# WCC-Analytics/sidecar

Measured on AMD Instinct MI355X. Metric: record-merges/sec (whole node) + rounds-to-converge wall time, H=32768 S=16, higher is better.
Workload: dtype int64

## Files before the change

sidecar_amd/csrc/gx_device.hpp:

```cpp
#pragma once
#include <hip/hip_runtime.h>
#include <stdint.h>

#include "../../include/gx.h"

#define GXD __device__ __forceinline__
#define GXHD __host__ __device__ __forceinline__

#define GX_GLOBAL __attribute__((address_space(1)))
typedef unsigned int gx_u32x4 __attribute__((ext_vector_type(4)));
template <class T>
GXD T gld(const T *p) {
  return *(const GX_GLOBAL T *)p;
}
typedef unsigned int gx_u32x3 __attribute__((ext_vector_type(3)));
template <class T>
GXD void gst(T *p, T v) {
  *(GX_GLOBAL T *)p = v;
}
GXD gx_u32x4 gld4(const void *p) { return *(const GX_GLOBAL gx_u32x4 *)p; }
GXD gx_u32x3 gld3(const void *p) { return *(const GX_GLOBAL gx_u32x3 *)p; }
GXD void gst4(void *p, gx_u32x4 v) { *(GX_GLOBAL gx_u32x4 *)p = v; }

struct grec {
// ... 51 lines not shown

struct Dev {
  gx_params p;
  int64_t epoch;
  uint32_t H, S, R, Q, A, L, SQ, DQ, K;
  uint32_t NG, KE;
  uint32_t KG;
  uint32_t lo, Hl, G, gid;
  uint32_t n_remote;
  uint32_t *msg_key;
  uint32_t *in_stamp;
  int64_t round, now;
  int partitioned;
  uint64_t *view;
  unsigned long long *minexp;
  uint8_t *own_status;
  gx_host_state *hs;
  gx_job *fifo;
  gx_sleeper *sleep;
  grec *dq;
  grec *arena;
  uint32_t *arena_len;
  uint32_t AW;
  uint32_t *arena_bits;
  grec *msg;
  uint64_t *msg_w0;
  uint32_t *msg_len;
  uint32_t *msg_dst;
  uint32_t DI;
  uint32_t DR;
  uint32_t *in_cnt;
  uint32_t *in_cnt_nx;
  uint4 *in_hdr;
  uint4 *in_ovf;
  grec *in_rec;
  uint32_t *work_cnt;
  uint32_t *wl_cnt, *wl_cnt_nx;
  uint32_t *ovf_cnt, *ovf_cnt_nx;
  uint32_t *work;
  uint32_t *mrec;
  grec *scan_list;
  uint32_t *scan_cnt;
  uint8_t *tick;
  uint16_t *sbytes;
  gx_server_times *srvt;
  int64_t *vlc;
  int32_t *ev_slot;
  gx_change_event *ev_log;
  uint32_t *ev_cnt;
  uint32_t ev_cap;
  DevCtr *ctr;
  gx_member *mem;
  int32_t *fd_dl;
  gx_fd_host *fdh;
  gx_fd_msg *fdm;
  uint32_t *fd_len;
  uint32_t *fd_peers;
  uint32_t *fd_np;
  uint64_t *fd_snap;
  int pair_split;
  uint64_t divS;
  uint32_t logS;
  int departures;
  uint32_t nblk_ae;
  uint64_t *snap;
  uint32_t snap_tag, snap_word;
// ... 145 lines not shown
    atomicMin(&d.ctr->first_drop[shard_id()][1], (unsigned long long)d.round);
}

GXD uint32_t li(const Dev &d, uint32_t v) { return v - d.lo; }
GXD uint32_t owner_of(const Dev &d, uint32_t r) { return d.S == 1 ? r : (uint32_t)__umul64hi(d.divS, (uint64_t)r); }
GXD bool owned_by(const Dev &d, uint32_t r, uint32_t o) { return r - o * d.S < d.S; }
GXD bool departed(const Dev &d, uint32_t u) { return d.departures && departed_at(d.p, d.round, u); }

GXD void wave_sync() {
  __builtin_amdgcn_fence(__ATOMIC_SEQ_CST, "wavefront");
  __builtin_amdgcn_wave_barrier();
}

#define GX_ERR_INBOX 1u
#define GX_WC_ERR 4
#define GX_WC_SCANS 5
#define GX_WC_N 8
#define GX_SNAP_QUIET 0xffffffffu
GXD uint32_t inbox_claim(const Dev &d, uint32_t vi) { return atomicAdd(&d.in_cnt[vi], 1u); }
GXD void inbox_header(const Dev &d, uint32_t vi, uint32_t pos, uint32_t key, uint32_t entry, uint32_t len,
                      uint32_t slot) {
  if (pos < d.DI) d.in_hdr[(size_t)vi * d.DI + pos] = make_uint4(key, entry, len, slot);
  else d.in_ovf[atomicAdd(d.ovf_cnt, 1u)] = make_uint4(key, entry, len, vi);
}
GXD void inbox_header(const Dev &d, uint32_t vi, uint32_t pos, uint32_t key, uint32_t entry, uint32_t len) {
  inbox_header(d, vi, pos, key, entry, len, pos);
}
GXD void inbox_put(const Dev &d, uint32_t vi, uint32_t key, uint32_t entry, uint32_t len) {
  inbox_header(d, vi, inbox_claim(d, vi), key, entry, len);
}
GXD grec *packet_recs(const Dev &d, uint32_t vi, uint32_t slot, uint32_t entry) {
  return slot < d.DR ? &d.in_rec[((size_t)vi * d.DR + slot) * d.p.packet_cap] : &d.msg[(size_t)entry * d.p.packet_cap];
}
GXD uint4 inbox_next(const Dev &d, uint32_t vi, int64_t after) {
  uint4 best = make_uint4(0xffffffffu, 0u, 0u, 0u);
  bool found = false;
  const uint32_t cnt = d.in_cnt[vi], n = cnt < d.DI ? cnt : d.DI;
  for (uint32_t i = 0; i < n; i++) {
    const uint4 h = d.in_hdr[(size_t)vi * d.DI + i];
    if ((int64_t)h.x > after && (!found || h.x < best.x)) {
      best = h;
      found = true;
    }
  }
  const uint32_t no = *d.ovf_cnt;
  for (uint32_t i = 0; i < no; i++) {
    const uint4 h = d.in_ovf[i];
    if (h.w == vi && (int64_t)h.x > after && (!found || h.x < best.x)) {
      best = make_uint4(h.x, h.y, h.z, 0xffffffffu);
      found = true;
    }
  }
  return best;
}
GXD void flag_live(const Dev &d, uint32_t vi, uint32_t n) { atomicAdd(&d.mrec[vi], n); }
GXD gx_member *memp(const Dev &d, uint32_t v, uint32_t m) { return &d.mem[(size_t)li(d, v) * d.H + m]; }
GXD int32_t *dlp(const Dev &d, uint32_t v, uint32_t m) { return &d.fd_dl[(size_t)li(d, v) * d.H + m]; }
GXD gx_fd_host *fdhp(const Dev &d, uint32_t v) { return &d.fdh[li(d, v)]; }
GXD bool reach(const Dev &d, uint32_t a, uint32_t b) {
  if (departed(d, a) || departed(d, b)) return false;
  return !(d.partitioned && ((a < d.H / 2) != (b < d.H / 2)));
}
GXD uint64_t *vrow(const Dev &d, uint32_t v) { return &d.view[(size_t)li(d, v) * d.R]; }
GXD gx_host_state *hst(const Dev &d, uint32_t v) { return &d.hs[li(d, v)]; }

GXD void set_slot(const Dev &d, Acc &a, uint32_t v, uint64_t *slot, uint64_t nw) {
  if (*slot != nw) {
    *slot = nw;
    a.changed = true;
    atomicMin(&d.minexp[li(d, v)], exp_time(d.p, nw));
  }
}

GXD bool locked_in(const Dev &d, uint32_t lockw) { return GX_LOCK_AT(lockw, d.round) != 0u; }
GXD bool host_locked(const Dev &d, uint32_t v) { return locked_in(d, gld(&hst(d, v)->lock)); }
GXD uint32_t lock_snap(uint32_t lockw, uint32_t flags, int64_t round, bool rw) {
  const uint32_t b = 1u << (round & 1), w = 16u << (round & 1);
  lockw = (lockw & ~b) | ((flags & 3u) ? b : 0u);
  return rw ? (lockw & ~w) | ((flags & 2u) ? w : 0u) : lockw;
}
#define GX_NOHOST 0xffffffffu
#define GX_LOCK_READERS_CLAIMED 2u
GXD bool ro_side(const Dev &d, uint32_t v) {
  const gx_host_state *h = hst(d, v);
  const uint32_t lw = gld(&h->lock);
// ... 608 lines not shown
```

sidecar_amd/csrc/gx_engine.hip:

```cpp
#include <hip/hip_runtime.h>

#include <math.h>
#include <stdio.h>
#include <stdlib.h>
#include <string.h>

#include <algorithm>
#include <chrono>
#include <deque>
#include <numeric>
#include <string>
#include <thread>
#include <type_traits>
#include <vector>


#define HIPCHK(x)                                                                          \
  do {                                                                                     \
    hipError_t _e = (x);                                                                   \
    if (_e != hipSuccess) {                                                                \
      fprintf(stderr, "gx: HIP error %s at %s:%d\n", hipGetErrorString(_e), __FILE__, __LINE__); \
      return GX_EIO;                                                                       \
    }                                                                                      \
  } while (0)
// ... 1030 lines not shown
  d.L = p->packet_cap + p->pending_cap;
  d.K = p->fanout;
  d.NG = p->gossip_messages > 1 ? p->gossip_messages : 1;
  d.KG = d.K * d.NG;
  d.KE = d.KG + (p->probe_piggyback ? 2u : 0u);
  d.divS = d.S > 1 ? ~0ull / d.S + 1 : 0;
  while ((1u << d.logS) < d.S) d.logS++;
  d.G = p->n_shards > 1 ? p->n_shards : 1;
  d.gid = d.G > 1 ? p->shard_id : 0;
  d.lo = (uint32_t)(((uint64_t)d.gid * d.H) / d.G);
  d.Hl = (uint32_t)(((uint64_t)(d.gid + 1) * d.H) / d.G) - d.lo;
  d.SQ = pow2_at_least(64 > d.KE * (p->retransmit_rounds + 1) ? 64 : d.KE * (p->retransmit_rounds + 1));
  d.DQ = pow2_at_least(d.L + p->pending_cap + 64);
  d.nblk_ae = (d.R + GX_DIGEST_SLOTS - 1) / GX_DIGEST_SLOTS;
  d.DI = p->inbox_slots ? p->inbox_slots : (d.NG > 1 ? GX_DI_MAX : 64);
  d.DR = d.DI < 8 ? d.DI : 8;
  d.sfilt = 1u;
  d.QW = 4 * nblk(d.Hl ? d.Hl : 1, 64);
  d.departures = p->depart_round >= 0 && p->depart_ppm;
  if (p->lock_model) {
    d.C = p->lock_buffer;
    d.PW = (d.H + 31) / 32;
    if (p->lock_readers) d.P = p->lock_defer_slots ? p->lock_defer_slots : 64;
    if (p->fd_handoff_shared) d.HQ = d.C > GX_LOCK_HANDLER_AT ? d.C - GX_LOCK_HANDLER_AT : 0;
  }
  e->scan_nch = 1;
  if (d.R >= 65536 && d.S >= 2 && 128 % d.S == 0)
    e->scan_nch = d.R / 32768 < 16 ? d.R / 32768 : 16;
  if (getenv("GX_KPROF"))
    e->kprof_n = (size_t)nblk(d.Hl, 64) * 4 * 8 + GX_KPROF_MERGE_N + 3ull * d.H;
  if (const char *qs = getenv("GX_QUIET_SEND")) e->quiet_send = strcmp(qs, "0") != 0;
  e->quiet_batch = GX_QUIET_BATCH;
  if (const char *qb = getenv("GX_QUIET_BATCH")) e->quiet_batch = (uint32_t)std::min(std::max(atol(qb), 1l), 1024l);
  if (d.G > 1) {
    e->nblk = d.nblk_ae;
    e->nmw = (e->nblk + 31) / 32;
  }
}

static int create_streams(gx_engine *e) {
  HIPCHK(hipStreamCreateWithFlags(&e->own_stream, hipStreamNonBlocking));
  e->stream = e->own_stream;
  HIPCHK(hipStreamCreateWithFlags(&e->side_stream, hipStreamNonBlocking));
  HIPCHK(hipEventCreateWithFlags(&e->side_start, hipEventDisableTiming));
  HIPCHK(hipEventCreateWithFlags(&e->side_done, hipEventDisableTiming));
  HIPCHK(hipHostMalloc((void **)&e->scan_snap, (2 + GX_QUIET_SLOTS) * sizeof(uint64_t), hipHostMallocMapped));
  HIPCHK(hipHostGetDevicePointer((void **)&e->scan_snap_dev, e->scan_snap, 0));
  e->scan_snap[0] = e->scan_snap[1] = ~0ull;
  for (int i = 0; i < GX_QUIET_SLOTS; i++) e->scan_snap[2 + i] = 0;
  return GX_OK;
}

#define DERIVED 0u
#define TAKE(...) GXTRY(e->mem.take(__VA_ARGS__))

static int create_buffers(gx_engine *e) {
  Dev &d = e->d;
  const gx_params *p = &d.p;
  hipStream_t s = e->stream;
  const size_t Hg = d.H, H = d.Hl, K = d.KE ? d.KE : 1;
  TAKE(GX_CK_VIEW, d.view, sizeof(uint64_t) * H * d.R);
  TAKE(GX_CK_OWN_STATUS, d.own_status, H * d.S);
  TAKE(GX_CK_HS, d.hs, sizeof(gx_host_state) * H);
  TAKE(GX_CK_FIFO, d.fifo, sizeof(gx_job) * H * d.Q);
  TAKE(GX_CK_SLEEP, d.sleep, sizeof(gx_sleeper) * H * d.SQ);
  TAKE(GX_CK_DQ, d.dq, sizeof(grec) * H * d.DQ);
  TAKE(GX_CK_ARENA, d.arena, sizeof(grec) * H * d.A * d.L);
  TAKE(GX_CK_ARENA_LEN, d.arena_len, sizeof(uint32_t) * H * d.A, 0, s);
  TAKE(GX_CK_ARENA_BITS, d.arena_bits, sizeof(uint32_t) * H * d.AW);
  TAKE(GX_CK_MSG, d.msg, sizeof(grec) * Hg * K * p->packet_cap);
  TAKE(GX_CK_MSG_W0, d.msg_w0, sizeof(uint64_t) * Hg * K * p->packet_cap);
  TAKE(GX_CK_MSG_LEN, d.msg_len, sizeof(uint32_t) * Hg * K, 0, s);
  TAKE(GX_CK_MSG_DST, d.msg_dst, sizeof(uint32_t) * Hg * K);
  TAKE(GX_CK_MSG_KEY, d.msg_key, sizeof(uint32_t) * Hg * K);
  TAKE(GX_CK_IN_CNT, e->in_cnt_buf, sizeof(uint32_t) * 2 * H, 0, s);
  TAKE(GX_CK_IN_HDR, d.in_hdr, sizeof(uint4) * H * d.DI);
  TAKE(GX_CK_IN_OVF, d.in_ovf, sizeof(uint4) * Hg * K);
  TAKE(GX_CK_IN_REC, d.in_rec, sizeof(grec) * H * d.DR * p->packet_cap);
  TAKE(GX_CK_WORK_CNT, d.work_cnt, sizeof(uint32_t) * GX_WC_N, 0, s);
  TAKE(DERIVED, d.quiet_w, sizeof(uint32_t) * 2 * d.QW, 0, s);
  TAKE(GX_CK_WORK, d.work, sizeof(uint32_t) * H);
  if (p->push_pull_mode == GX_PP_INITIATE && d.G < 2) {
    TAKE(DERIVED, e->pp_dev, sizeof(uint32_t) * 2 * Hg);
    TAKE(DERIVED, e->pp_prow, sizeof(int32_t) * Hg, 0xff, s);
  }
  TAKE(GX_CK_MREC, d.mrec, sizeof(uint32_t) * H, 0, s);
  TAKE(GX_CK_MINEXP, d.minexp, sizeof(unsigned long long) * H);
  TAKE(GX_CK_SCAN_LIST, d.scan_list, sizeof(grec) * H * d.L);
  TAKE(GX_CK_SCAN_CNT, d.scan_cnt, sizeof(uint32_t) * H);
  if (e->scan_nch > 1) {
    TAKE(DERIVED, e->scan_tmp, sizeof(grec) * H * e->scan_nch * d.L);
    TAKE(DERIVED, e->scan_chunk, sizeof(ScanChunk) * H * e->scan_nch);
  }
  TAKE(GX_CK_TICK, d.tick, H, 0, s);
  TAKE(GX_CK_SBYTES, d.sbytes, sizeof(uint16_t) * d.R);
  TAKE(GX_CK_SRVT, d.srvt, sizeof(gx_server_times) * H * Hg);
  TAKE(GX_CK_VLC, d.vlc, sizeof(int64_t) * H);
  TAKE(DERIVED, d.ev_slot, sizeof(int32_t) * H, 0xff, s);
  TAKE(GX_CK_CTR, d.ctr, sizeof(DevCtr), 0, s);
  if (p->fd_enable) {
    TAKE(GX_CK_MEM, d.mem, sizeof(gx_member) * H * Hg);
    TAKE(GX_CK_FD_DL, d.fd_dl, sizeof(int32_t) * H * Hg);
    TAKE(GX_CK_FDH, d.fdh, sizeof(gx_fd_host) * H);
    TAKE(GX_CK_FDM, d.fdm, sizeof(gx_fd_msg) * Hg * K * p->fd_msg_cap);
    TAKE(GX_CK_FD_LEN, d.fd_len, sizeof(uint32_t) * Hg * K, 0, s);
    TAKE(GX_CK_FD_PEERS, d.fd_peers, sizeof(uint32_t) * H * K);
    TAKE(GX_CK_FD_NP, d.fd_np, sizeof(uint32_t) * H);
    if (p->fd_push_pull_state) TAKE(GX_CK_FD_SNAP, d.fd_snap, sizeof(uint64_t) * H * Hg);
  }
// ... 394 lines not shown
```

sidecar_amd/csrc/gx_kernels.hpp:

```cpp
#pragma once
#include "gx_device.hpp"

GXD unsigned long long block_excl_scan64(unsigned long long x, unsigned long long *s_wave,
                                         unsigned long long &total) {
  uint32_t lane = threadIdx.x & 63, w = threadIdx.x >> 6, nw = (blockDim.x + 63) >> 6;
  unsigned long long incl = x;
  for (int o = 1; o < 64; o <<= 1) {
    unsigned long long y = __shfl_up(incl, o, 64);
    if ((int)lane >= o) incl += y;
  }
  if (lane == 63) s_wave[w] = incl;
  __syncthreads();
  unsigned long long off = 0, tot = 0;
  for (uint32_t i = 0; i < nw; i++) {
    unsigned long long c = s_wave[i];
    if (i < w) off += c;
    tot += c;
  }
  __syncthreads();
  total = tot;
  return off + incl - x;
}
GXD uint32_t fld(unsigned long long x, int i) { return (uint32_t)((x >> (16 * i)) & 0xffffu); }

// ... 1296 lines not shown
GXD uint32_t shard_of_d(const Dev &d, uint32_t v) {
  uint32_t g = (uint32_t)(((uint64_t)v * d.G) / d.H);
  while (g > 0 && (uint32_t)(((uint64_t)g * d.H) / d.G) > v) g--;
  while (g + 1 < d.G && (uint32_t)(((uint64_t)(g + 1) * d.H) / d.G) <= v) g++;
  return g;
}
GXD uint32_t *ob_slot_hdr(const Dev &d, uint32_t slot) {
  return reinterpret_cast<uint32_t *>(d.ob_buf + (size_t)slot * (16u + 16u * d.p.packet_cap));
}
static_assert(sizeof(PlanCall) >= 17 * sizeof(uint32_t), "a PlanCall slot holds a team's 16 peers and their count");
#define GX_NOSLOT 0xffffffffu
#define GX_NOSLOT_W0 0xfffffffeu
GXD bool w0_fwd(const Dev &d, uint32_t slot, uint32_t tick, uint32_t key, uint32_t v) {
  return slot == GX_NOSLOT_W0 && tick != 2 && !owned_by(d, key, v);
}

GXD grec plan_item(const Dev &d, const PlanCall &c, uint32_t i) {
  grec g;
  g.pad = 0;
  if (c.kind == GX_JOB_SEND) {
    const grec s = c.list[i];
    g.w = s.w + c.bw;
    g.r = s.r;
  } else if (c.kind == GX_JOB_EXPIRE) {
    g.w = c.bw;
    g.r = c.rb + (c.emask ? nth_set_bit(c.emask, i) : i);
  } else {
    g.w = c.bw;
    g.r = c.rb;
  }
  return g;
}

template <int T, bool QUIET = false>
GXD void send_planned(const Dev &d, Acc &a, uint32_t idx, gx_host_state &hs, gx_job *pjs, PlanCall *pl,
                      const uint32_t *peers, uint32_t np, unsigned long long &kb, unsigned long long &kl,
                      uint32_t npf0 = 0) {
  constexpr int PLAN_Q = PLAN_RECS / T;
  const uint32_t lane = threadIdx.x & 63, tl = lane & (T - 1), tw = lane / T;
  const bool lead = tl == 0;
  const uint64_t tmask = T == 64 ? ~0ull : ((1ull << T) - 1ull);
  const uint32_t u = d.lo + idx, cap = d.p.packet_cap, mask = d.DQ - 1;
  grec *dq = &d.dq[(size_t)idx * d.DQ];
  grec *const arena_t = &d.arena[(size_t)idx * d.A * d.L];
  grec *const msg_t = &d.msg[(size_t)idx * d.KE * cap];
  uint64_t *const w0_t = &d.msg_w0[(size_t)idx * d.KE * cap];
  const int64_t t_stale = d.now - d.p.tombstone_lifespan_ns - d.p.stale_fudge_ns;
  const int64_t t_gc = d.now - d.p.tombstone_lifespan_ns;
  uint32_t pf0 = hs.fifo_head, npf = npf0;
  uint32_t j = 0, n = 0;
  bool stop = np == 0;
  unsigned fm = 0, fs = 0, nlines = 0;
  GX_SPLIT_DECL
  const bool lmod = QUIET || d.p.lock_model != 0;
  constexpr int NR = (16 + T - 1) / T;
  const bool direct = !QUIET && d.ob_buf != nullptr;
  uint32_t osl[NR];
  uint32_t emit = 0;
#pragma unroll
  for (int r = 0; r < NR; r++) osl[r] = GX_NOSLOT;
  uint32_t og[NR], rk[NR], ksrc[NR], krun[NR], lc[NR], lb[NR], le[NR];
  if (direct) {
    unsigned long long pend[NR];
#pragma unroll
    for (int r = 0; r < NR; r++) {
      const uint32_t jj = (uint32_t)r * T + tl;
      og[r] = jj < np && peers[jj] - d.lo >= d.Hl ? shard_of_d(d, peers[jj]) : d.G;
      pend[r] = __ballot(og[r] < d.G);
      rk[r] = ksrc[r] = krun[r] = lc[r] = 0;
    }
    for (;;) {
      int r0 = -1;
#pragma unroll
      for (int r = NR - 1; r >= 0; r--) r0 = pend[r] ? r : r0;
      if (r0 < 0) break;
      unsigned long long p0 = pend[0];
      uint32_t g0 = og[0];
#pragma unroll
      for (int r = 1; r < NR; r++) {
        p0 = r == r0 ? pend[r] : p0;
        g0 = r == r0 ? og[r] : g0;
      }
      const uint32_t src = (uint32_t)__builtin_ctzll(p0);
      const uint32_t gs = (uint32_t)__shfl((int)g0, (int)src, 64);
      uint32_t acc = 0;
#pragma unroll
      for (int r = 0; r < NR; r++) {
// ... 149 lines not shown
        const uint32_t nn = c.m + hs.dq_len;
        l = nn < cap ? nn : cap;
        c.head = hs.dq_head;
        if (l < c.m) {
          c.push = c.m - l;
          c.nh = (c.head - c.push) & mask;
          any_push = true;
        } else {
          c.nh = (c.head + (l - c.m)) & mask;
        }
        hs.dq_head = c.nh;
        hs.dq_len = nn - l;
        if (hs.dq_len > d.p.pending_cap) {
          if (lead) a.c[C_PDROP] += hs.dq_len - d.p.pending_cap;
          hs.dq_len = d.p.pending_cap;
        }
        if (l && lead) {
          a.c[C_PACKETS]++;
          a.c[C_RECSENT] += l;
          const uint32_t lb = l < c.m ? l : c.m;
          const bool filt = c.row && !(lmod && c.lk);
          if (c.lk & 2u) {
            a.c[C_LOCK_DROP] += l;
          } else {
            kb += 16ull * ((c.kind == GX_JOB_SEND ? lb : 0u) + (l - lb)) + (filt ? 8ull * l : 0ull);
          }
          if (filt) fm += l;
          if (c.lk) {
            a.locked = true;
            if (!lmod) a.c[C_LOCKED_MERGES] += l;
          }
        }
      }
      c.l = l;
      c.lpre = tot;
      if (l) {
        if (c.oslot != GX_NOSLOT) emit |= 1u << j;
        if constexpr (QUIET) {
          if (c.push) cp = c;
        } else {
          if (lead) pl[nc] = c;
        }
        nc++;
        if (!(c.lk & 2u)) tot += l;
      }
      const bool pushed = c.push != 0;
      if (l == 0) {
        if (n == 0 && d.p.gossip_stop_on_empty) stop = true;
        j++;
        n = 0;
      } else if (++n == d.NG) {
        j++;
        n = 0;
      }
      if (j >= np) stop = true;
      if (pushed) break;
    }
    if (nc == 0) break;
    if constexpr (QUIET) {
#ifndef GX_SEND_SPLIT
      if (j <= PLAN_CH) {
        GX_KP(5);
        GX_KP(6);
      }
#endif
      GX_SPLIT(0);
      for (uint32_t qq = (tl - cp.nh) & (T - 1); qq < cp.push; qq += T) {
        dq[(cp.nh + qq) & mask] = plan_item(d, cp, cp.l + qq);
        kb += 16;
      }
      GX_SPLIT(3);
      continue;
    }
    wave_sync();
#ifndef GX_SEND_SPLIT
    if (j <= PLAN_CH) GX_KP(5);
#endif
// ... 91 lines not shown
        }
        if (live) {
          grec g;
          g.w = w[q];
          g.r = r[q];
          g.pad = 0;
          const uint32_t xo = (c.x - idx * d.KE) * cap + rank;
          grec *to = c.oslot != GX_NOSLOT ? reinterpret_cast<grec *>(ob_slot_hdr(d, c.oslot) + 4) + rank : &msg_t[xo];
          gst_rec(to, g);
          if (filt) gst(&w0_t[xo], w0[q]);
        }
        run += (uint32_t)__popcll(lm);
      }
    }
#pragma unroll
    for (int kk = 1; kk < PLAN_CH; kk++)
      if (lp[kk] == tot) cb[kk] = run;
    uint32_t stored_all = 0;
#ifndef GX_SEND_SPLIT
    if (j <= PLAN_CH) GX_KP(6);
#endif
    GX_SPLIT(1);
    if (tl < nc) {
      const PlanCall &c = pl[tl];
      uint32_t stored = 0;
#pragma unroll
      for (int kk = 0; kk < PLAN_CH; kk++) {
        const uint32_t end = kk + 1 < PLAN_CH && (uint32_t)(kk + 1) < nc ? cb[kk + 1] : run;
        stored = (uint32_t)kk == tl ? end - cb[kk] : stored;
      }
      const uint32_t rv = c.peer - d.lo;
      if (!c.row) stored = c.l;
      if (c.lk & 2u) stored = 0;
      d.msg_len[c.x] = stored;
      d.msg_dst[c.x] = c.peer;
      if (c.oslot != GX_NOSLOT)
        *reinterpret_cast<uint4 *>(ob_slot_hdr(d, c.oslot)) = make_uint4(c.key, c.peer, stored, 0u);
      if (c.row && stored) {
        inbox_header(d, rv, inbox_claim(d, rv), c.key, c.x, stored, lmod && c.lk ? GX_NOSLOT : GX_NOSLOT_W0);
        flag_live(d, rv, stored);
      }
      stored_all = stored + ((c.row && stored) ? 2u : 0u);
    }
    kb += 16ull * stored_all;
    GX_SPLIT(2);
    if (any_push) {
      for (uint32_t k = 0; k < nc; k++) {
        const PlanCall &c = pl[k];
        for (uint32_t qq = (tl - c.nh) & (T - 1); qq < c.push; qq += T) {
          dq[(c.nh + qq) & mask] = plan_item(d, c, c.l + qq);
          kb += 16;
        }
      }
      __threadfence_block();
    }
    wave_sync();
    GX_SPLIT(3);
  }
  GX_SPLIT_FLUSH();
#pragma unroll
  for (int r = 0; r < NR; r++)
    if (osl[r] != GX_NOSLOT && !((emit >> ((uint32_t)r * T + tl)) & 1u))
      *reinterpret_cast<uint4 *>(ob_slot_hdr(d, osl[r])) = make_uint4(GX_SLOT_EMPTY, 0u, 0u, 0u);
  a.c[C_GOSSIP_MERGES] += fm;
  kl += nlines;
  a.c[C_STALE] += fs;
}

GXD bool filt_used(const Dev &d, uint32_t pos) { return d.sfilt && pos != 0xffffffffu; }
#define PLAN_PEERS(QUIET) ((QUIET) ? 0 : PLAN_CH)
template <int T, bool FWD, int SW>
GXD uint32_t quiet_tick(const Dev &d, Acc &a, uint32_t idx, gx_host_state &hs, gx_sleeper *sj, gx_job *pj,
                        uint32_t *peers) {
  const uint32_t tl = threadIdx.x & (T - 1), o = d.lo + idx;
  const bool lead = tl == 0;
// ... 400 lines not shown
      const unsigned long long n = wave_sum((unsigned long long)cross[c]);
      if ((threadIdx.x & 63) == 0 && n) atomicAdd(&d.probe_x[c], n);
    }
  }
}

template <bool K32>
GXD uint64_t bitonic64(uint64_t x, uint32_t lane) {
#pragma unroll
  for (uint32_t k = 2; k <= 64; k <<= 1) {
#pragma unroll
    for (uint32_t j = k >> 1; j > 0; j >>= 1) {
      uint64_t o;
      if (K32) o = (uint32_t)__shfl_xor((uint32_t)x, (int)j, 64);
      else o = __shfl_xor(x, (int)j, 64);
      bool keep_min = ((lane & j) == 0) == ((lane & k) == 0);
      x = keep_min ? (o < x ? o : x) : (o > x ? o : x);
    }
  }
  return x;
}

GXD uint32_t rdl(uint32_t x, uint32_t l) { return (uint32_t)__builtin_amdgcn_readlane((int)x, (int)l); }

GXD void merge_inbox_serial(const Dev &d, uint32_t vi, bool lockd = false, uint32_t nbuf = 0) {
  Acc a;
  const uint32_t v = d.lo + vi, cnt = d.in_cnt[vi];
  int64_t after = -1;
  unsigned long long recs = 0;
  grec *lkb = d.lkb ? &d.lkb[(size_t)vi * d.C] : nullptr;
  if (lockd) {
    uint32_t nb = GX_LOCK_BUF(d.hs[vi].lock);
    const uint32_t capv = pipe_cap(d, vi, d.hs[vi].lock);
    for (uint32_t n = 0; n < cnt; n++) {
      const uint4 h = inbox_next(d, vi, after);
      after = h.x;
      const grec *pk = packet_recs(d, vi, h.w, h.y);
      for (uint32_t x = 0; x < h.z; x++) {
        if (nb < capv) {
          lkb[nb++] = pk[x];
          a.c[C_LOCK_BUF]++;
        } else {
          a.c[C_LOCK_DROP]++;
        }
      }
      recs += h.z;
    }
    d.hs[vi].lock = (d.hs[vi].lock & ((1u << GX_LOCK_BUF_SHIFT) - 1u)) | nb << GX_LOCK_BUF_SHIFT;
    kbytes(d, GX_K_MERGE, 32ull * recs + 16ull * cnt + 4, 0);
    for (int i = 0; i < C_NCTR; i++) ctr_atomic(d, i, a.c[i]);
    return;
  }
  for (uint32_t k = 0; k < nbuf; k++) add_entry(d, a, v, lkb[k], SRC_GOSSIP);
  const unsigned m0 = a.c[C_GOSSIP_MERGES], s0 = a.c[C_STALE];
  if (nbuf) {
    a.c[C_LOCK_DRAIN] += nbuf;
    d.hs[vi].lock &= (1u << GX_LOCK_BUF_SHIFT) - 1u;
  }
  for (uint32_t n = 0; n < cnt; n++) {
    const uint4 h = inbox_next(d, vi, after);
    after = h.x;
    const grec *pk = packet_recs(d, vi, h.w, h.y);
    for (uint32_t x = 0; x < h.z; x++) add_entry(d, a, v, pk[x], SRC_GOSSIP);
    recs += h.z;
  }
  recs += nbuf;
  a.c[C_GOSSIP_MERGES] = m0;
  a.c[C_STALE] = s0;
  kbytes(d, GX_K_MERGE, 28ull * recs + 16ull * cnt + 4, recs);
  for (int i = 0; i < C_NCTR; i++) ctr_atomic(d, i, a.c[i]);
  if (a.changed) mark_change(d);
}

#define INBOX_PREFETCH 8
#define MERGE_WAVES 4
#define MSET 512
#define MSET_EMPTY 0xffffffffu
GXD uint32_t mset_slot(uint32_t key) { return (key * 0x9E3779B1u) >> (32 - 9); }
GXD bool mset_has(const uint32_t *set, uint32_t key) {
  for (uint32_t h = mset_slot(key), n = 0; n < MSET; n++, h = (h + 1) & (MSET - 1)) {
    const uint32_t x = set[h];
    if (x == key) return true;
// ... 10 lines not shown
struct MergeLds {
  uint4 hdr[GX_DI_MAX];
  uint32_t pst[GX_DI_MAX];
  uint64_t accw[64];
  uint32_t wset[MSET];
  uint8_t accf[64], chg[64], prev[64];
};
template <bool K32, bool EV>
GXD void merge_receiver(const Dev &d, const uint32_t vi, MergeLds &L) {
  uint4 *s_hdr = L.hdr;
  uint8_t *s_accf = L.accf, *s_chg = L.chg, *s_prev = L.prev;
  uint64_t *s_accw = L.accw;
  const uint32_t lane = threadIdx.x & 63, v = d.lo + vi;
  const uint32_t npre = d.DI < INBOX_PREFETCH ? d.DI : INBOX_PREFETCH;
  uint4 hd = lane < npre ? d.in_hdr[(size_t)vi * d.DI + lane] : make_uint4(0u, 0u, 0u, 0u);
  const uint32_t deg = d.in_cnt[vi];
  uint32_t lw = 0, nbuf = 0;
  bool lockd = false;
  if (d.p.lock_model) {
    lw = __builtin_amdgcn_readfirstlane(d.hs[vi].lock);
    lockd = locked_in(d, lw);
    nbuf = lockd || departed(d, v) ? 0u : GX_LOCK_BUF(lw);
  }
  if (deg == 0 && nbuf == 0) return;
  if (deg > d.DI) {
    if (lane == 0) merge_inbox_serial(d, vi, lockd, nbuf);
    return;
  }
  const bool wide = deg > 64;
  uint4 sh = make_uint4(0u, 0u, 0u, 0u);
  uint32_t pstart = 0, total = 0;
  if (!wide) {
    if (deg > npre && lane >= npre && lane < deg) hd = d.in_hdr[(size_t)vi * d.DI + lane];
    const uint32_t hkey = lane < deg ? hd.x : 0xffffffffu;
    uint32_t hrank = 0;
    for (uint32_t j = 0; j < deg; j++) hrank += rdl(hkey, j) < hkey || (rdl(hkey, j) == hkey && j < lane);
    if (lane < deg) s_hdr[hrank] = hd;
    wave_sync();
    sh = lane < deg ? s_hdr[lane] : make_uint4(0u, 0u, 0u, 0u);
    uint32_t incl = sh.z;
#pragma unroll
    for (int o = 1; o < 64; o <<= 1) {
      uint32_t y = __shfl_up(incl, o, 64);
      if ((int)lane >= o) incl += y;
    }
    pstart = incl - sh.z;
    total = __shfl(incl, 63, 64);
  } else {
    constexpr int HPL = GX_DI_MAX / 64;
    uint4 hw[HPL];
#pragma unroll
    for (int c = 0; c < HPL; c++) {
      const uint32_t j = lane + 64u * c;
      hw[c] = j < deg ? (j < npre ? hd : d.in_hdr[(size_t)vi * d.DI + j]) : make_uint4(0u, 0u, 0u, 0u);
      if (j < deg) L.pst[j] = hw[c].x;
    }
    wave_sync();
    uint32_t rk[HPL];
#pragma unroll
    for (int c = 0; c < HPL; c++) rk[c] = 0;
    for (uint32_t j = 0; j < deg; j++) {
      const uint32_t kj = L.pst[j];
#pragma unroll
      for (int c = 0; c < HPL; c++) {
        const uint32_t me = lane + 64u * c;
        rk[c] += kj < hw[c].x || (kj == hw[c].x && j < me);
      }
    }
#pragma unroll
    for (int c = 0; c < HPL; c++)
      if (lane + 64u * c < deg) s_hdr[rk[c]] = hw[c];
    wave_sync();
    for (uint32_t c0 = 0; c0 < deg; c0 += 64) {
      const uint32_t j = c0 + lane;
      const uint32_t ln = j < deg ? s_hdr[j].z : 0u;
      uint32_t incl = ln;
#pragma unroll
      for (int o = 1; o < 64; o <<= 1) {
        uint32_t y = __shfl_up(incl, o, 64);
        if ((int)lane >= o) incl += y;
      }
      if (j < deg) L.pst[j] = total + incl - ln;
      total += __shfl(incl, 63, 64);
    }
    wave_sync();
  }
  const uint32_t vtick = d.tick[vi];
// ... 14 lines not shown
  }
  const grec *lkb = nbuf ? &d.lkb[(size_t)vi * d.C] : nullptr;
  const uint32_t ntot = nbuf + total;
  auto load_recs = [&](uint32_t tb, grec &g, uint32_t &fslot, uint64_t &fw0) {
    uint32_t i = tb + lane;
    g.w = 0;
    g.r = INV;
    g.pad = 0;
    fw0 = 0;
    fslot = 0;
    if (i < nbuf) {
      g = gld_rec(&lkb[i]);
      return;
    }
    i -= nbuf;
    if (i < total) {
      uint32_t lo = 0, hi = deg;
      while (hi - lo > 1) {
        const uint32_t mid = (lo + hi) >> 1;
        if (L.pst[mid] <= i) lo = mid;
        else hi = mid;
      }
      const uint4 hk = s_hdr[lo];
      const uint32_t off = i - L.pst[lo];
      fslot = hk.w;
      g = packet_recs(d, vi, hk.w, hk.y)[off];
      if (hk.w == GX_NOSLOT_W0) fw0 = d.msg_w0[(size_t)hk.y * d.p.packet_cap + off];
    }
  };
  if (lockd) {
    const uint32_t capv = pipe_cap(d, vi, lw), nb0 = GX_LOCK_BUF(lw), room_l = capv > nb0 ? capv - nb0 : 0u;
    const uint32_t keep = total < room_l ? total : room_l;
    grec *dst = &d.lkb[(size_t)vi * d.C + nb0];
    for (uint32_t t0 = 0; t0 < keep; t0 += 64) {
      grec g;
      uint32_t fs;
      uint64_t fw;
      load_recs(t0, g, fs, fw);
      if (t0 + lane < keep) gst_rec(&dst[t0 + lane], g);
    }
    if (lane == 0) {
      d.hs[vi].lock = (lw & ((1u << GX_LOCK_BUF_SHIFT) - 1u)) | (nb0 + keep) << GX_LOCK_BUF_SHIFT;
      ctr_atomic(d, C_LOCK_BUF, keep);
      ctr_atomic(d, C_LOCK_DROP, total - keep);
      kbytes(d, GX_K_MERGE, 32ull * keep + 16ull * deg + 4, 0);
    }
    wave_sync();
    return;
  }
  const bool track = ntot > 64;
  if (track)
    for (uint32_t q = lane; q < MSET; q += 64) L.wset[q] = MSET_EMPTY;
  uint32_t nset = 0;
  grec gc, gn;
  uint32_t fsc, fsn = 0;
  uint64_t fwc, fwn = 0;
  load_recs(0, gc, fsc, fwc);
  gn.w = 0;
  gn.r = INV;
  gn.pad = 0;
  if (64 < ntot) load_recs(64, gn, fsn, fwn);
  wave_sync();
  unsigned long long *kpm = kprof_merge(d);
  unsigned long long ph[5] = {0, 0, 0, 0, 0}, tk = 0;
  uint32_t c_dstale = 0;
  for (uint32_t t0 = 0; t0 < ntot; t0 += 64) {
    if (kpm) tk = __builtin_amdgcn_s_memtime();
    const uint32_t i = t0 + lane;
    const bool valid = i < ntot;
    uint32_t key = INV;
    uint64_t val = 0, w0 = 0;
    bool rd = false;
    if (valid) {
      key = gc.r;
      val = gc.w;
      bool fwd = w0_fwd(d, fsc, vtick, key, v);
      if (fwd && t0 > 0) fwd = nset <= MSET / 2 && !mset_has(L.wset, key);
      rd = !fwd;
// ... 350 lines not shown
    const uint32_t ok = n_retx < room ? n_retx : room;
    if (n_retx) {
      d.hs[vi].fifo_tail = tail0 + n_retx;
      d.hs[vi].fifo_stored = st0 + ok;
    }
    if (mcmax) d.vlc[vi] = ts_of(s_accw[mcmax - 1]);
    if (EV && evk >= 0) d.ev_cnt[evk] = ev0 + n_ev;
    ctr_atomic(d, C_CHG, c_chg);
    kbytes(d, GX_K_MERGE, 12ull * total + 8ull * (total + c_wr) + 16ull * ok + 16ull * deg + 4, total);
    ctr_atomic(d, C_GOSSIP_ACC, c_acc);
    ctr_atomic(d, C_RETX, n_retx);
    ctr_atomic(d, C_QDEFER, n_retx - ok);
    if (c_wr) {
      mark_change(d);
      atomicMin(&d.minexp[vi], mexp);
    }
  }
  wave_sync();
  return true;
}

#ifndef MERGE_WPE_GM
#define MERGE_WPE_GM 4
#endif
#ifndef LOCK_RPL
#define LOCK_RPL 4
#endif
template <int SEG>
GXD bool lock_append_seg(const Dev &d, uint32_t vi, bool act) {
  const uint32_t lane = threadIdx.x & 63, sl = lane & (SEG - 1), sb = lane & ~(uint32_t)(SEG - 1);
  const uint32_t deg = act ? d.in_cnt[vi] : 0u;
  const uint32_t lw = act ? d.hs[vi].lock : 0u;
  uint4 hd = d.in_hdr[(size_t)vi * d.DI + (sl < d.DI ? sl : 0u)];
  if (deg > (uint32_t)SEG || deg > d.DI) return false;
  if (sl >= deg) hd = make_uint4(0xffffffffu, 0u, 0u, 0u);
  uint32_t start = 0, total = 0;
  for (uint32_t j = 0; j < (uint32_t)SEG; j++) {
    const uint32_t kj = (uint32_t)__shfl((int)hd.x, (int)(sb + j), 64);
    const uint32_t lj = (uint32_t)__shfl((int)hd.z, (int)(sb + j), 64);
    const bool before = j < deg && (kj < hd.x || (kj == hd.x && j < sl));
    start += before ? lj : 0u;
    total += j < deg ? lj : 0u;
  }
  const uint32_t capv = pipe_cap(d, vi, lw), nb0 = GX_LOCK_BUF(lw), room = capv > nb0 ? capv - nb0 : 0u;
  const uint32_t keep = total < room ? total : room;
  grec *dst = act ? &d.lkb[(size_t)vi * d.C + nb0] : d.lkb;
  for (uint32_t o0 = 0; o0 < keep; o0 += SEG * LOCK_RPL) {
    grec g[LOCK_RPL];
#pragma unroll
    for (int q = 0; q < LOCK_RPL; q++) {
      const uint32_t o = o0 + sl + SEG * q;
      uint32_t entry = 0, slot = 0, off = 0;
      for (uint32_t j = 0; j < deg; j++) {
        const uint32_t sj = (uint32_t)__shfl((int)start, (int)(sb + j), 64);
        const uint32_t lj = (uint32_t)__shfl((int)hd.z, (int)(sb + j), 64);
        const uint32_t ej = (uint32_t)__shfl((int)hd.y, (int)(sb + j), 64);
        const uint32_t wj = (uint32_t)__shfl((int)hd.w, (int)(sb + j), 64);
        if (o >= sj && o < sj + lj) {
          entry = ej;
          slot = wj;
          off = o - sj;
        }
      }
      g[q] = gld_rec(&packet_recs(d, vi, slot, entry)[off]);
    }
#pragma unroll
    for (int q = 0; q < LOCK_RPL; q++) {
      const uint32_t o = o0 + sl + SEG * q;
      if (o < keep) gst_rec(&dst[o], g[q]);
    }
  }
  if (act && sl == 0 && deg) {
    d.hs[vi].lock = (lw & ((1u << GX_LOCK_BUF_SHIFT) - 1u)) | (nb0 + keep) << GX_LOCK_BUF_SHIFT;
    ctr_atomic(d, C_LOCK_BUF, keep);
    ctr_atomic(d, C_LOCK_DROP, total - keep);
    kbytes(d, GX_K_MERGE, 32ull * keep + 16ull * deg + 4, 0);
  }
  return true;
}

#ifndef GX_LOCK_APPEND_WPE
#define GX_LOCK_APPEND_WPE 8
#endif
__global__ __launch_bounds__(256) __attribute__((amdgpu_waves_per_eu(GX_LOCK_APPEND_WPE))) void k_lock_append(Dev d) {
  const uint32_t vi = (blockIdx.x * 256u + threadIdx.x) >> 4;
  bool act = false;
  if (vi < d.Hl) act = d.mrec[vi] != 0 && locked_in(d, d.hs[vi].lock);
  if (__ballot(act) == 0) return;
  const bool ok = lock_append_seg<16>(d, act ? vi : 0u, act);
  if (act && ok && (threadIdx.x & 15) == 0) d.mrec[vi] = 0;
}

#define MERGE_NR 64
#define MERGE_NONE 0xffffffffu
template <bool K32, bool EV, int NR = MERGE_NR, int WPE = 3>
__global__ __launch_bounds__(64 * MERGE_WAVES) __attribute__((amdgpu_waves_per_eu(WPE))) void k_merge_seg(Dev d) {
  static_assert(NR <= 64, "one routing lane per receiver");
  __shared__ MergeLds s_l[MERGE_WAVES];
  __shared__ uint32_t s_it[NR][4];
  __shared__ uint32_t s_ty[NR];
  __shared__ uint32_t s_fb[NR], s_n[2];
  const uint32_t wv = threadIdx.x >> 6, lane = threadIdx.x & 63;
  const uint32_t r0 = blockIdx.x * NR;
  if (wv == 0) {
    const uint32_t vi = r0 + lane;
    uint32_t t = 0;
    if (lane < (uint32_t)NR && vi < d.Hl) t = d.mrec[vi];
    if (t) d.mrec[vi] = 0;
    if (lane < (uint32_t)NR)
// ... 2156 lines not shown
```

Before: 4.153 billion.

## Send compact packet descriptors for lock-buffered expire/retx records instead of full records

Result: no change. 4.114 billion (-0.9%).

```diff
diff --git a/profiles/lock_desc/pmc_sum.py b/profiles/lock_desc/pmc_sum.py
--- /dev/null
+++ b/profiles/lock_desc/pmc_sum.py
@@ -0,0 +1,28 @@
+import csv
+import json
+import sys
+
+FIRST, LAST = 9, 28
+
+if __name__ == "__main__":
+    label, counter, path = sys.argv[1:4]
+    rows = {}
+    with open(path) as f:
+        for r in csv.DictReader(f):
+            if r["Counter_Name"] == counter:
+                k = int(r["Dispatch_Id"])
+                name, v = rows.get(k, (r["Kernel_Name"], 0.0))
+                rows[k] = (name, v + float(r["Counter_Value"]))
+    scale = 1024.0 * (2 if counter == "FETCH_SIZE" else 1)
+    rnd, out = -1, {"k_send": [0, 0.0], "k_lock_append": [0, 0.0]}
+    for k in sorted(rows):
+        name, v = rows[k]
+        if "k_send" in name:
+            rnd += 1
+        base = "k_send" if "k_send" in name else "k_lock_append" if "k_lock_append" in name else None
+        if base and FIRST <= rnd <= LAST:
+            out[base][0] += 1
+            out[base][1] += v * scale
+    print(json.dumps({"lib": label, "counter": counter, "rounds": f"{FIRST}..{LAST}",
+                      **{k: {"launches": n, "MB": round(b / 1e6, 2), "MB_per_launch": round(b / 1e6 / max(1, n), 3)}
+                         for k, (n, b) in out.items()}}))
diff --git a/profiles/lock_desc/rounds.py b/profiles/lock_desc/rounds.py
--- /dev/null
+++ b/profiles/lock_desc/rounds.py
@@ -0,0 +1,12 @@
+import os
+import sys
+
+sys.path.insert(0, os.getcwd())
+import bench
+from sidecar_amd.abi import load_product
+
+if __name__ == "__main__":
+    e = bench.make_engine(load_product(), "cfg5", 0x5EED, 0)
+    for _ in range(int(sys.argv[1])):
+        e.run_rounds(1)
+    print(e.round, e.stats()["lock_buffered"])
diff --git a/profiles/lock_desc/stretch.py b/profiles/lock_desc/stretch.py
--- /dev/null
+++ b/profiles/lock_desc/stretch.py
@@ -0,0 +1,29 @@
+import json
+import os
+import sys
+import time
+
+sys.path.insert(0, os.getcwd())
+import bench
+from sidecar_amd.abi import load_product
+
+if __name__ == "__main__":
+    lib = load_product()
+    e = bench.make_engine(lib, "cfg5", 0x5EED, 0)
+    e.run_rounds(9)
+    t0, s0 = e.timing(), e.stats()
+    e.run_rounds(2)
+    spans = {}
+    for first in (11, 21, 31, 41):
+        assert e.round == first
+        a = time.perf_counter()
+        e.run_rounds(9)
+        spans[f"{first}..{first + 8}"] = round((time.perf_counter() - a) * 1e6 / 9, 2)
+        e.run_rounds(1 if first < 41 else 0)
+    t1, s1 = e.timing(), e.stats()
+    print(json.dumps({"lib": sys.argv[1], "lock_desc_env": os.environ.get("GX_LOCK_DESC"), "us_per_round": spans,
+                      "rounds_9_48": {"send_bytes": t1["send"]["bytes"] - t0["send"]["bytes"],
+                                      "merge_bytes": t1["merge"]["bytes"] - t0["merge"]["bytes"],
+                                      "lock_buffered": s1["lock_buffered"] - s0["lock_buffered"],
+                                      "lock_drops": s1["lock_drops"] - s0["lock_drops"],
+                                      "records_sent": s1["records_sent"] - s0["records_sent"]}}))
diff --git a/sidecar_amd/csrc/gx_device.hpp b/sidecar_amd/csrc/gx_device.hpp
--- a/sidecar_amd/csrc/gx_device.hpp
+++ b/sidecar_amd/csrc/gx_device.hpp
@@ -107,6 +107,8 @@
   uint32_t *in_cnt;
   uint32_t *in_cnt_nx;
   uint4 *in_hdr;
+  uint4 *in_desc;
+  uint32_t lock_desc;
   uint4 *in_ovf;
   grec *in_rec;
   uint32_t *work_cnt;
@@ -318,14 +320,18 @@
 GXD grec *packet_recs(const Dev &d, uint32_t vi, uint32_t slot, uint32_t entry) {
   return slot < d.DR ? &d.in_rec[((size_t)vi * d.DR + slot) * d.p.packet_cap] : &d.msg[(size_t)entry * d.p.packet_cap];
 }
-GXD uint4 inbox_next(const Dev &d, uint32_t vi, int64_t after) {
+#define GX_NOSLOT_DESC 0xfffffffdu
+#define GX_OVF_DESC 0x80000000u
+GXD uint4 inbox_next(const Dev &d, uint32_t vi, int64_t after, uint32_t *pos = nullptr) {
   uint4 best = make_uint4(0xffffffffu, 0u, 0u, 0u);
   bool found = false;
+  uint32_t at = 0xffffffffu;
   const uint32_t cnt = d.in_cnt[vi], n = cnt < d.DI ? cnt : d.DI;
   for (uint32_t i = 0; i < n; i++) {
     const uint4 h = d.in_hdr[(size_t)vi * d.DI + i];
     if ((int64_t)h.x > after && (!found || h.x < best.x)) {
       best = h;
+      at = i;
       found = true;
     }
   }
@@ -333,10 +339,12 @@
   for (uint32_t i = 0; i < no; i++) {
     const uint4 h = d.in_ovf[i];
     if (h.w == vi && (int64_t)h.x > after && (!found || h.x < best.x)) {
-      best = make_uint4(h.x, h.y, h.z, 0xffffffffu);
+      best = make_uint4(h.x, h.y, h.z & ~GX_OVF_DESC, (h.z & GX_OVF_DESC) ? GX_NOSLOT_DESC : 0xffffffffu);
+      at = 0xffffffffu;
       found = true;
     }
   }
+  if (pos) *pos = at;
   return best;
 }
 GXD void flag_live(const Dev &d, uint32_t vi, uint32_t n) { atomicAdd(&d.mrec[vi], n); }
diff --git a/sidecar_amd/csrc/gx_engine.hip b/sidecar_amd/csrc/gx_engine.hip
--- a/sidecar_amd/csrc/gx_engine.hip
+++ b/sidecar_amd/csrc/gx_engine.hip
@@ -1086,6 +1086,8 @@
   if (const char *qs = getenv("GX_QUIET_SEND")) e->quiet_send = strcmp(qs, "0") != 0;
   e->quiet_batch = GX_QUIET_BATCH;
   if (const char *qb = getenv("GX_QUIET_BATCH")) e->quiet_batch = (uint32_t)std::min(std::max(atol(qb), 1l), 1024l);
+  d.lock_desc = p->lock_model ? 1u : 0u;
+  if (const char *ld = getenv("GX_LOCK_DESC")) d.lock_desc = d.lock_desc && strcmp(ld, "0") != 0;
   if (d.G > 1) {
     e->nblk = d.nblk_ae;
     e->nmw = (e->nblk + 31) / 32;
@@ -1129,6 +1131,7 @@
   TAKE(GX_CK_MSG_KEY, d.msg_key, sizeof(uint32_t) * Hg * K);
   TAKE(GX_CK_IN_CNT, e->in_cnt_buf, sizeof(uint32_t) * 2 * H, 0, s);
   TAKE(GX_CK_IN_HDR, d.in_hdr, sizeof(uint4) * H * d.DI);
+  if (d.lock_desc) TAKE(DERIVED, d.in_desc, sizeof(uint4) * 2 * H * d.DI);
   TAKE(GX_CK_IN_OVF, d.in_ovf, sizeof(uint4) * Hg * K);
   TAKE(GX_CK_IN_REC, d.in_rec, sizeof(grec) * H * d.DR * p->packet_cap);
   TAKE(GX_CK_WORK_CNT, d.work_cnt, sizeof(uint32_t) * GX_WC_N, 0, s);
diff --git a/sidecar_amd/csrc/gx_kernels.hpp b/sidecar_amd/csrc/gx_kernels.hpp
--- a/sidecar_amd/csrc/gx_kernels.hpp
+++ b/sidecar_amd/csrc/gx_kernels.hpp
@@ -1352,6 +1352,50 @@
   return g;
 }
 
+#define GX_DESC_MASK 0x100u
+struct PktDesc {
+  uint4 a, b;
+};
+GXD PktDesc desc_of(const PlanCall &c) {
+  PktDesc ds;
+  ds.a = make_uint4((uint32_t)c.bw, (uint32_t)(c.bw >> 32), c.rb, c.kind | (c.emask ? GX_DESC_MASK : 0u));
+  ds.b = make_uint4((uint32_t)c.emask, (uint32_t)(c.emask >> 32), 0u, 0u);
+  return ds;
+}
+GXD bool desc_masked(const PktDesc &ds) { return (ds.a.w & GX_DESC_MASK) != 0; }
+GXD uint32_t desc_bytes(const PktDesc &ds) { return desc_masked(ds) ? 32u : 16u; }
+GXD grec desc_item(const PktDesc &ds, uint32_t i) {
+  const uint64_t emask = (uint64_t)ds.b.x | ((uint64_t)ds.b.y << 32);
+  grec g;
+  g.w = (uint64_t)ds.a.x | ((uint64_t)ds.a.y << 32);
+  g.r = ds.a.z + (desc_masked(ds) ? nth_set_bit(emask, i) : i);
+  g.pad = 0;
+  return g;
+}
+GXD uint4 *desc_at(const Dev &d, uint32_t vi, uint32_t pos, uint32_t entry) {
+  return pos < d.DI ? &d.in_desc[((size_t)vi * d.DI + pos) * 2] : reinterpret_cast<uint4 *>(&d.msg[(size_t)entry * d.p.packet_cap]);
+}
+GXD PktDesc packet_desc(const Dev &d, uint32_t vi, uint32_t pos, uint32_t entry) {
+  const uint4 *p = desc_at(d, vi, pos, entry);
+  PktDesc ds;
+  ds.a = p[0];
+  ds.b = make_uint4(0u, 0u, 0u, 0u);
+  if (desc_masked(ds)) ds.b = p[1];
+  return ds;
+}
+GXD grec packet_rec(const Dev &d, uint32_t vi, uint32_t slot, uint32_t entry, const PktDesc &ds, uint32_t x) {
+  if (slot == GX_NOSLOT_DESC) return desc_item(ds, x);
+  return gld_rec(&packet_recs(d, vi, slot, entry)[x]);
+}
+GXD void inbox_header_desc(const Dev &d, uint32_t vi, uint32_t pos, uint32_t key, uint32_t entry, uint32_t len,
+                           const PktDesc &ds) {
+  uint4 *p = desc_at(d, vi, pos, entry);
+  p[0] = ds.a;
+  if (desc_masked(ds)) p[1] = ds.b;
+  if (pos < d.DI) d.in_hdr[(size_t)vi * d.DI + pos] = make_uint4(key, entry, len, GX_NOSLOT_DESC);
+  else d.in_ovf[atomicAdd(d.ovf_cnt, 1u)] = make_uint4(key, entry, len | GX_OVF_DESC, vi);
+}
+
 template <int T, bool QUIET = false>
 GXD void send_planned(const Dev &d, Acc &a, uint32_t idx, gx_host_state &hs, gx_job *pjs, PlanCall *pl,
                       const uint32_t *peers, uint32_t np, unsigned long long &kb, unsigned long long &kl,
@@ -1373,6 +1417,7 @@
   unsigned fm = 0, fs = 0, nlines = 0;
   GX_SPLIT_DECL
   const bool lmod = QUIET || d.p.lock_model != 0;
+  const bool dsc_ok = !QUIET && lmod && d.lock_desc && cap >= 2;
   constexpr int NR = (16 + T - 1) / T;
   const bool direct = !QUIET && d.ob_buf != nullptr;
   uint32_t osl[NR];
@@ -1588,6 +1633,7 @@
           }
         }
       }
+      if (dsc_ok && c.row && c.lk == 1u && l && l <= c.m && (c.kind == GX_JOB_EXPIRE || c.kind == GX_JOB_RETX)) c.lk |= 4u;
       c.l = l;
       c.lpre = tot;
       if (l) {
@@ -1598,7 +1644,7 @@
           if (lead) pl[nc] = c;
         }
         nc++;
-        if (!(c.lk & 2u)) tot += l;
+        if (!(c.lk & 6u)) tot += l;
       }
       const bool pushed = c.push != 0;
       if (l == 0) {
@@ -1756,15 +1802,20 @@
       const uint32_t rv = c.peer - d.lo;
       if (!c.row) stored = c.l;
       if (c.lk & 2u) stored = 0;
+      const bool dsc = (c.lk & 4u) != 0;
+      if (dsc) stored = c.l;
       d.msg_len[c.x] = stored;
       d.msg_dst[c.x] = c.peer;
       if (c.oslot != GX_NOSLOT)
         *reinterpret_cast<uint4 *>(ob_slot_hdr(d, c.oslot)) = make_uint4(c.key, c.peer, stored, 0u);
-      if (c.row && stored) {
+      if (dsc) {
+        inbox_header_desc(d, rv, inbox_claim(d, rv), c.key, c.x, stored, desc_of(c));
+        flag_live(d, rv, stored);
+      } else if (c.row && stored) {
         inbox_header(d, rv, inbox_claim(d, rv), c.key, c.x, stored, lmod && c.lk ? GX_NOSLOT : GX_NOSLOT_W0);
         flag_live(d, rv, stored);
       }
-      stored_all = stored + ((c.row && stored) ? 2u : 0u);
+      stored_all = (dsc ? (c.emask ? 2u : 1u) : stored) + ((c.row && stored) ? 2u : 0u);
     }
     kb += 16ull * stored_all;
     GX_SPLIT(2);
@@ -2231,22 +2282,27 @@
   if (lockd) {
     uint32_t nb = GX_LOCK_BUF(d.hs[vi].lock);
     const uint32_t capv = pipe_cap(d, vi, d.hs[vi].lock);
+    unsigned long long moved = 0;
     for (uint32_t n = 0; n < cnt; n++) {
-      const uint4 h = inbox_next(d, vi, after);
+      uint32_t pos;
+      const uint4 h = inbox_next(d, vi, after, &pos);
       after = h.x;
-      const grec *pk = packet_recs(d, vi, h.w, h.y);
+      const bool dsc = h.w == GX_NOSLOT_DESC;
+      PktDesc ds;
+      ds.a = ds.b = make_uint4(0u, 0u, 0u, 0u);
+      if (dsc) ds = packet_desc(d, vi, pos, h.y);
       for (uint32_t x = 0; x < h.z; x++) {
         if (nb < capv) {
-          lkb[nb++] = pk[x];
+          lkb[nb++] = packet_rec(d, vi, h.w, h.y, ds, x);
           a.c[C_LOCK_BUF]++;
         } else {
           a.c[C_LOCK_DROP]++;
         }
       }
-      recs += h.z;
+      moved += dsc ? desc_bytes(ds) + 16ull * h.z : 32ull * h.z;
     }
     d.hs[vi].lock = (d.hs[vi].lock & ((1u << GX_LOCK_BUF_SHIFT) - 1u)) | nb << GX_LOCK_BUF_SHIFT;
-    kbytes(d, GX_K_MERGE, 32ull * recs + 16ull * cnt + 4, 0);
+    kbytes(d, GX_K_MERGE, moved + 16ull * cnt + 4, 0);
     for (int i = 0; i < C_NCTR; i++) ctr_atomic(d, i, a.c[i]);
     return;
   }
@@ -2323,6 +2379,7 @@
   uint32_t pstart = 0, total = 0;
   if (!wide) {
     if (deg > npre && lane >= npre && lane < deg) hd = d.in_hdr[(size_t)vi * d.DI + lane];
+    if (hd.w == GX_NOSLOT_DESC) hd.y = lane;
     const uint32_t hkey = lane < deg ? hd.x : 0xffffffffu;
     uint32_t hrank = 0;
     for (uint32_t j = 0; j < deg; j++) hrank += rdl(hkey, j) < hkey || (rdl(hkey, j) == hkey && j < lane);
@@ -2344,6 +2401,7 @@
     for (int c = 0; c < HPL; c++) {
       const uint32_t j = lane + 64u * c;
       hw[c] = j < deg ? (j < npre ? hd : d.in_hdr[(size_t)vi * d.DI + j]) : make_uint4(0u, 0u, 0u, 0u);
+      if (hw[c].w == GX_NOSLOT_DESC) hw[c].y = j;
       if (j < deg) L.pst[j] = hw[c].x;
     }
     wave_sync();
@@ -2424,18 +2482,34 @@
     const uint32_t capv = pipe_cap(d, vi, lw), nb0 = GX_LOCK_BUF(lw), room_l = capv > nb0 ? capv - nb0 : 0u;
     const uint32_t keep = total < room_l ? total : room_l;
     grec *dst = &d.lkb[(size_t)vi * d.C + nb0];
+    uint32_t nld = 0;
     for (uint32_t t0 = 0; t0 < keep; t0 += 64) {
-      grec g;
-      uint32_t fs;
-      uint64_t fw;
-      load_recs(t0, g, fs, fw);
-      if (t0 + lane < keep) gst_rec(&dst[t0 + lane], g);
-    }
+      const uint32_t i = t0 + lane;
+      if (i < keep) {
+        uint32_t lo = 0, hi = deg;
+        while (hi - lo > 1) {
+          const uint32_t mid = (lo + hi) >> 1;
+          if (L.pst[mid] <= i) lo = mid;
+          else hi = mid;
+        }
+        const uint4 hk = s_hdr[lo];
+        PktDesc dk;
+        dk.a = dk.b = make_uint4(0u, 0u, 0u, 0u);
+        if (hk.w == GX_NOSLOT_DESC) dk = packet_desc(d, vi, hk.y, 0u);
+        else nld++;
+        gst_rec(&dst[i], packet_rec(d, vi, hk.w, hk.y, dk, i - L.pst[lo]));
+      }
+    }
+    nld = (uint32_t)wave_sum(nld);
+    uint32_t nds = 0;
+    for (uint32_t j = lane; j < deg; j += 64)
+      if (s_hdr[j].w == GX_NOSLOT_DESC) nds += desc_bytes(packet_desc(d, vi, s_hdr[j].y, 0u));
+    nds = (uint32_t)wave_sum(nds);
     if (lane == 0) {
       d.hs[vi].lock = (lw & ((1u << GX_LOCK_BUF_SHIFT) - 1u)) | (nb0 + keep) << GX_LOCK_BUF_SHIFT;
       ctr_atomic(d, C_LOCK_BUF, keep);
       ctr_atomic(d, C_LOCK_DROP, total - keep);
-      kbytes(d, GX_K_MERGE, 32ull * keep + 16ull * deg + 4, 0);
+      kbytes(d, GX_K_MERGE, 16ull * keep + 16ull * nld + nds + 16ull * deg + 4, 0);
     }
     wave_sync();
     return;
@@ -2852,8 +2926,15 @@
   const uint32_t deg = act ? d.in_cnt[vi] : 0u;
   const uint32_t lw = act ? d.hs[vi].lock : 0u;
   uint4 hd = d.in_hdr[(size_t)vi * d.DI + (sl < d.DI ? sl : 0u)];
+  PktDesc ds;
+  ds.a = ds.b = make_uint4(0u, 0u, 0u, 0u);
+  if (d.lock_desc) ds.a = *desc_at(d, vi, sl < d.DI ? sl : 0u, 0u);
   if (deg > (uint32_t)SEG || deg > d.DI) return false;
   if (sl >= deg) hd = make_uint4(0xffffffffu, 0u, 0u, 0u);
+  const bool dsc = hd.w == GX_NOSLOT_DESC;
+  const bool masks = __ballot(dsc && desc_masked(ds)) != 0;
+  if (masks && dsc && desc_masked(ds)) ds.b = desc_at(d, vi, sl, 0u)[1];
+  if (!dsc) ds.a.w = 0u;
   uint32_t start = 0, total = 0;
   for (uint32_t j = 0; j < (uint32_t)SEG; j++) {
     const uint32_t kj = (uint32_t)__shfl((int)hd.x, (int)(sb + j), 64);
@@ -2867,34 +2948,58 @@
   grec *dst = act ? &d.lkb[(size_t)vi * d.C + nb0] : d.lkb;
   for (uint32_t o0 = 0; o0 < keep; o0 += SEG * LOCK_RPL) {
     grec g[LOCK_RPL];
+    uint32_t kp[LOCK_RPL];
+    bool ld = false;
+    constexpr uint32_t GX_NOPKT = 0x200u;
 #pragma unroll
     for (int q = 0; q < LOCK_RPL; q++) {
       const uint32_t o = o0 + sl + SEG * q;
-      uint32_t entry = 0, slot = 0, off = 0;
+      kp[q] = GX_NOPKT;
       for (uint32_t j = 0; j < deg; j++) {
         const uint32_t sj = (uint32_t)__shfl((int)start, (int)(sb + j), 64);
         const uint32_t lj = (uint32_t)__shfl((int)hd.z, (int)(sb + j), 64);
-        const uint32_t ej = (uint32_t)__shfl((int)hd.y, (int)(sb + j), 64);
         const uint32_t wj = (uint32_t)__shfl((int)hd.w, (int)(sb + j), 64);
-        if (o >= sj && o < sj + lj) {
-          entry = ej;
-          slot = wj;
-          off = o - sj;
-        }
-      }
-      g[q] = gld_rec(&packet_recs(d, vi, slot, entry)[off]);
+        if (o >= sj && o < sj + lj) kp[q] = j | (wj == GX_NOSLOT_DESC ? 0x100u : 0u);
+      }
+      ld |= o < keep && !(kp[q] & 0x100u);
+    }
+    if (__ballot(ld)) {
+#pragma unroll
+      for (int q = 0; q < LOCK_RPL; q++) {
+        const bool rec = kp[q] < 0x100u;
+        const uint32_t k = sb + (rec ? kp[q] : sl);
+        const uint32_t sk = (uint32_t)__shfl((int)start, (int)k, 64);
+        const uint32_t ek = (uint32_t)__shfl((int)hd.y, (int)k, 64);
+        const uint32_t wk = (uint32_t)__shfl((int)hd.w, (int)k, 64);
+        const uint32_t o = o0 + sl + SEG * q;
+        g[q] = gld_rec(&packet_recs(d, vi, rec ? wk : 0u, rec ? ek : 0u)[rec ? o - sk : 0u]);
+      }
     }
 #pragma unroll
     for (int q = 0; q < LOCK_RPL; q++) {
       const uint32_t o = o0 + sl + SEG * q;
-      if (o < keep) gst_rec(&dst[o], g[q]);
-    }
-  }
+      const uint32_t k = sb + ((kp[q] & 0x100u) ? (kp[q] & 0xffu) : sl);
+      const uint32_t sk = (uint32_t)__shfl((int)start, (int)k, 64);
+      PktDesc dk;
+      dk.a.x = (uint32_t)__shfl((int)ds.a.x, (int)k, 64);
+      dk.a.y = (uint32_t)__shfl((int)ds.a.y, (int)k, 64);
+      dk.a.z = (uint32_t)__shfl((int)ds.a.z, (int)k, 64);
+      dk.a.w = masks ? (uint32_t)__shfl((int)ds.a.w, (int)k, 64) : 0u;
+      dk.b.x = masks ? (uint32_t)__shfl((int)ds.b.x, (int)k, 64) : 0u;
+      dk.b.y = masks ? (uint32_t)__shfl((int)ds.b.y, (int)k, 64) : 0u;
+      dk.b.z = dk.b.w = 0u;
+      if (o < keep) gst_rec(&dst[o], (kp[q] & 0x100u) ? desc_item(dk, o - sk) : g[q]);
+    }
+  }
+  const uint32_t kept = sl < deg && keep > start ? (keep - start < hd.z ? keep - start : hd.z) : 0u;
+  uint32_t rd = sl < deg ? (dsc ? desc_bytes(ds) : 16u * kept) : 0u;
+#pragma unroll
+  for (int o = SEG / 2; o > 0; o >>= 1) rd += (uint32_t)__shfl_xor((int)rd, o, SEG);
   if (act && sl == 0 && deg) {
     d.hs[vi].lock = (lw & ((1u << GX_LOCK_BUF_SHIFT) - 1u)) | (nb0 + keep) << GX_LOCK_BUF_SHIFT;
     ctr_atomic(d, C_LOCK_BUF, keep);
     ctr_atomic(d, C_LOCK_DROP, total - keep);
-    kbytes(d, GX_K_MERGE, 32ull * keep + 16ull * deg + 4, 0);
+    kbytes(d, GX_K_MERGE, 16ull * keep + rd + 16ull * deg + 4, 0);
   }
   return true;
 }
```
